# vita-epfl/CrowdNav

Measured on NVIDIA H100. Metric: env-steps/sec at 5 humans × batched envs; 500-case success/collision parity, higher is better.
Workload: dtype f64 state + f32 ORCA solver

## Files before the change

crowdnav_b200/build.py:

```python
#!/usr/bin/env python
import os
import shutil
import subprocess
import sys

HERE = os.path.dirname(os.path.abspath(__file__))
CSRC = os.path.join(HERE, 'csrc')
TARGET = os.path.join(CSRC, 'libcrowdsim_b200.so')
SOURCES = ['step_kernel.cu', 'reset_kernel.cu', 'pack_kernel.cu', 'times_kernel.cu', 'record_kernel.cu']
HEADERS = ['crowdsim_common.cuh', 'orca_device.cuh', 'step_flat.cuh', 'step_multi.cuh', 'step_mid.cuh', 'orca_spec.cuh', 'rotate.cuh', 'step_args.cuh', 'occupancy.cuh', os.path.join('..', '..', 'include', 'crowdsim_b200.h')]
NVCC_FLAGS = ['-gencode', 'arch=compute_90a,code=sm_90a', '-O3', '-lineinfo', '--fmad=false',
              '-prec-div=true', '-prec-sqrt=true', '-ftz=false', '-std=c++17',
              '-Xcompiler', '-fPIC', '-shared', '-cudart', 'shared', '--threads', '4']


def _nvcc():
    for c in (shutil.which('nvcc'), '/usr/local/cuda/bin/nvcc'):
        if c and os.path.exists(c):
            return c
    raise RuntimeError('nvcc not found')


def _stale():
    if not os.path.exists(TARGET):
        return True
    t = os.path.getmtime(TARGET)
    deps = [os.path.join(CSRC, s) for s in SOURCES + HEADERS] + [__file__]
    return any(os.path.exists(d) and os.path.getmtime(d) > t for d in deps)


def build(force=False, verbose=False, extra=()):
    srcs = [os.path.join(CSRC, s) for s in SOURCES]
    if force or _stale():
        cmd = [_nvcc()] + NVCC_FLAGS + list(extra) + srcs + ['-o', TARGET]
        if verbose:
            print(' '.join(cmd))
        subprocess.check_call(cmd)
    return TARGET


if __name__ == '__main__':
    v = '--verbose' in sys.argv
    build(force='--force' in sys.argv, verbose=v, extra=['-Xptxas', '-v'] if v else [])
    print(TARGET)
```

crowdnav_b200/csrc/step_kernel.cu:

```cuda
#include "crowdsim_common.cuh"

namespace cs {

unsigned long long g_launches = 0;
int g_force_generic = 0;

}
#include "step_args.cuh"
#include "step_flat.cuh"
#include "step_multi.cuh"
#include "step_mid.cuh"
namespace cs {

#ifndef CS_MID_MINBLOCKS
#define CS_MID_MINBLOCKS 5
#endif

template <bool MID>
__global__ void __launch_bounds__(MID ? 128 : 256, MID ? CS_MID_MINBLOCKS : 1) step_kernel(const __grid_constant__ StepArgs A)
{
    extern __shared__ __align__(16) unsigned char smem[];
    __shared__ int s_qcount;
    const int T = blockDim.x, tid = threadIdx.x;
    const int N = A.N, L = A.L;
    const KParams &k = A.k;
    const Stage s = carve_stage(smem, A.EPB, L, k.nb_alloc, T);
    if (MID && tid == 0) s_qcount = 0;

    const int le = tid / L, a = tid - le * L;
    const int e = blockIdx.x * A.EPB + le;
    const bool is_robot = (a == N);
    bool live = (e < A.B);
    if (live && A.st.active) live = (A.st.active[e] != 0);

    double2 pos = make_double2(0, 0), vel = pos, goal = pos, attr = pos;
    double theta = 0, gtime = 0;
    if (live) {
        if (!is_robot) {
            const size_t i = (size_t)e * N + a;
            pos = ld2(A.st.h_pos, i); vel = ld2(A.st.h_vel, i); goal = ld2(A.st.h_goal, i); attr = ld2(A.st.h_attr, i);
        } else {
            pos = ld2(A.st.r_pos, e); vel = ld2(A.st.r_vel, e); goal = ld2(A.st.r_goal, e); attr = ld2(A.st.r_attr, e);
            gtime = A.st.g_time[e];
            if (k.robot_policy == CROWDSIM_ROBOT_EXTERNAL_ROT) theta = A.st.r_theta[e];
        }
    }
    stage_agent(s, k, tid, pos, vel, attr.x);
    __syncthreads();

    orca::V2 nv = orca::mk(0.f, 0.f);
    const bool solve = live && (!is_robot || k.robot_policy == CROWDSIM_ROBOT_ORCA) && !(A.act_only && !is_robot);
    if constexpr (MID) nv = mid_solve<kMidM>(s, k, solve, le, a, N, L, pos, goal, attr.y, tid, T, s.lines, &s_qcount);
    else if (solve) nv = orca_predict(s, k, le, a, N, L, pos, goal, attr.y, tid, T);

    if (A.act_only) {
        if (live && is_robot) st2(A.io.action_out, e, make_double2((double)nv.x, (double)nv.y));
        return;
    }

    double ax = 0, ay = 0;
    double2 rvel = make_double2(0, 0);
    if (live && is_robot) {
        if (k.robot_policy == CROWDSIM_ROBOT_ORCA) { ax = (double)nv.x; ay = (double)nv.y; rvel = make_double2(ax, ay); }
        else {
            const double2 act = ld2(A.io.action, e); ax = act.x; ay = act.y;
            if (k.robot_policy == CROWDSIM_ROBOT_EXTERNAL_ROT) rvel = make_double2(ax * cos(ay + theta), ax * sin(ay + theta));
            else rvel = act;
        }
        s.act[le] = rvel;
    }
    __syncthreads();

    const double dt = k.time_step;
    if (live && !is_robot) {
        const double2 rp = s.pos64[le * L + N], ra = s.act[le];
        const double px = pos.x - rp.x, py = pos.y - rp.y;
        const double vx = vel.x - ra.x, vy = vel.y - ra.y;
        const double ex = px + vx * dt, ey = py + vy * dt;
        s.closest[tid] = point_to_segment_dist0(px, py, ex, ey) - attr.x - s.rad64[le * L + N];
    }
    __syncthreads();

    const bool env_ok = (e < A.B);
    int install = 0;
    if (is_robot && env_ok) {
        bool done = false;
        if (live) {
            double dmin = __longlong_as_double(0x7ff0000000000000LL); bool collision = false;
            for (int i = 0; i < N; ++i) {
                const double c = s.closest[le * L + i];
                if (c < 0) { collision = true; break; }
                else if (c < dmin) dmin = c;
            }
            double npx, npy, nvx, nvy;
            if (k.robot_policy != CROWDSIM_ROBOT_EXTERNAL_ROT) { npx = pos.x + ax * dt; npy = pos.y + ay * dt; nvx = ax; nvy = ay; }
            else { const double th = theta + ay; npx = pos.x + cos(th) * ax * dt; npy = pos.y + sin(th) * ax * dt; nvx = nvy = 0; }
            const bool reaching_goal = norm2(npx - goal.x, npy - goal.y) < attr.x;

            double reward; int info;
            if (gtime >= k.time_limit - 1) { reward = 0; done = true; info = CROWDSIM_INFO_TIMEOUT; }
            else if (collision) { reward = k.collision_penalty; done = true; info = CROWDSIM_INFO_COLLISION; }
            else if (reaching_goal) { reward = k.success_reward; done = true; info = CROWDSIM_INFO_REACHGOAL; }
            else if (dmin < k.discomfort_dist) { reward = (dmin - k.discomfort_dist) * k.discomfort_penalty_factor * dt; done = false; info = CROWDSIM_INFO_DANGER; }
            else { reward = 0; done = false; info = CROWDSIM_INFO_NOTHING; }

            if (k.robot_policy == CROWDSIM_ROBOT_EXTERNAL_ROT) {
                double nth = fmod(theta + ay, 2 * CS_PI); if (nth < 0) nth += 2 * CS_PI;
                if (!A.lookahead) A.st.r_theta[e] = nth;
                nvx = ax * cos(nth); nvy = ax * sin(nth);
            }
            const double ntime = gtime + dt;
            if (!A.lookahead) {
                st2(A.st.r_pos, e, make_double2(npx, npy));
                st2(A.st.r_vel, e, make_double2(nvx, nvy));
                A.st.g_time[e] = ntime;
            }
            if (A.io.action_out) st2(A.io.action_out, e, make_double2(nvx, nvy));
            A.io.reward[e] = reward; A.io.dmin[e] = dmin; A.io.done[e] = done ? 1 : 0; A.io.info[e] = (uint8_t)info;

            if (A.has_ep) {
                const crowdsim_episodes &ep = A.ep;
                const int t = ep.ep_steps[e];
                const double disc = (t < ep.discount_len) ? ep.discount[t] : 0.0;
                const double ret = ep.ep_return[e] + disc * reward;
                int tc = ep.ep_too_close[e]; double mds = ep.ep_min_dist_sum[e];
                if (info == CROWDSIM_INFO_DANGER) { tc += 1; mds += dmin; ep.ep_too_close[e] = tc; ep.ep_min_dist_sum[e] = mds; }
                ep.ep_return[e] = ret; ep.ep_steps[e] = t + 1;
                if (done) {
                    const int c = ep.ep_case[e];
                    if (c >= 0) {
                        ep.res_info[c] = (uint8_t)info; ep.res_steps[c] = t + 1;
                        ep.res_time[c] = (info == CROWDSIM_INFO_TIMEOUT) ? k.time_limit : ntime;
                        ep.res_return[c] = ret; ep.res_too_close[c] = tc; ep.res_min_dist_sum[c] = mds;
                        if (ep.res_final_rpos) st2(ep.res_final_rpos, c, make_double2(npx, npy));
                    }
                    if (A.st.active && !A.has_ar) A.st.active[e] = 0;
                }
            }
        }
        if (A.has_ar) install = ar_decide(A, e, ld_relaxed_u8(A.ar.n_state + e), live && done, !live && A.ar.want[e] != 0);
    }
    if (A.has_ar) {
        if (is_robot) s.closest[le * L + N] = (double)install;
        __syncthreads();
        install = (s.closest[le * L + N] != 0.0) && env_ok;
        if (install) {
            if (is_robot) ar_install_robot(A, e);
            else {
                ar_install_human(A, e, N, a);
                if (A.io.obs32) { const double2 np_ = ld2_cg(A.ar.n_h_pos, (size_t)e * N + a); reinterpret_cast<float4 *>(A.io.obs32)[(size_t)e * N + a] = make_float4((float)np_.x, (float)np_.y, 0.f, 0.f); }
            }
        }
        __syncthreads();
        if (install && is_robot) st_release_u8(A.ar.n_state + e, CROWDSIM_SLOT_EMPTY);
    }
    if (live && !is_robot && !install) {
        const double hx = (double)nv.x, hy = (double)nv.y;
        const size_t i = (size_t)e * N + a;
        const double2 np_ = make_double2(pos.x + hx * dt, pos.y + hy * dt);
        if (A.lookahead) { st2(A.la_pos, i, np_); st2(A.la_vel, i, make_double2(hx, hy)); return; }
        st2(A.st.h_pos, i, np_);
        st2(A.st.h_vel, i, make_double2(hx, hy));
        if (A.io.obs32) reinterpret_cast<float4 *>(A.io.obs32)[i] = make_float4((float)np_.x, (float)np_.y, nv.x, nv.y);
    }
}


template <int N>
__global__ void __launch_bounds__(128) orca_act_kernel(const __grid_constant__ StepArgs A)
{
    using namespace orca;
    constexpr int M = N, T = 128;
    __shared__ float s_l[4 * M][T], s_pj[4 * M][T];
    const int e = blockIdx.x * T + threadIdx.x, tid = threadIdx.x;
    if (e >= A.B) return;
    if (A.st.active && !A.st.active[e]) return;
    const KParams &k = A.k;
    const double2 pos = ld2(A.st.r_pos, e), vel = ld2(A.st.r_vel, e), goal = ld2(A.st.r_goal, e), attr = ld2(A.st.r_attr, e);
    const double gvx = goal.x - pos.x, gvy = goal.y - pos.y;
    const double speed = norm2(gvx, gvy);
    const V2 pref = mk((float)((speed > 1) ? gvx / speed : gvx), (float)((speed > 1) ? gvy / speed : gvy));
    const V2 p = mk((float)pos.x, (float)pos.y), v = mk((float)vel.x, (float)vel.y);
    const float r = (float)(attr.x + 0.01 + k.robot_safety_space), max_speed = (float)attr.y;
    V2 hp[M], hv[M]; float hr[M]; float dsq[M]; bool inr[M]; int id[M], src[M];
    #pragma unroll
    for (int c = 0; c < M; ++c) {
        const size_t i = (size_t)e * N + c;
        const double2 q = ld2(A.st.h_pos, i), w = ld2(A.st.h_vel, i), at = ld2(A.st.h_attr, i);
        hp[c] = mk((float)q.x, (float)q.y); hv[c] = mk((float)w.x, (float)w.y); hr[c] = (float)(at.x + 0.01 + k.robot_safety_space);
        dsq[c] = abssq(p - hp[c]); inr[c] = (k.max_neighbors > 0) && dsq[c] < sqr(k.neighbor_dist); id[c] = c;
    }
    int nl = neighbour_order<M>(dsq, inr, id, src);
    nl = nl < k.max_neighbors ? nl : k.max_neighbors;
    RegLines<M> R; bool valid[M];
    #pragma unroll
    for (int kk = 0; kk < M; ++kk) {
        valid[kk] = kk < nl; R.p[kk] = mk(0.f, 0.f); R.d[kk] = mk(0.f, 0.f);
        V2 qp = hp[0], qv = hv[0]; float qr = hr[0];
        #pragma unroll
        for (int c = 1; c < M; ++c) if (src[kk] == c) { qp = hp[c]; qv = hv[c]; qr = hr[c]; }
        if (valid[kk]) make_line_sel(p, v, r, qp, qv, qr, k.inv_time_horizon, k.inv_time_step, R.p[kk], R.d[kk]);
    }
    V2 cand[M]; bool feas[M];
    lp1_all<M, M>(R, valid, max_speed, pref, false, cand, feas);
    V2 nv = mk(0.f, 0.f);
    const int fail = lp2_scan<M, M>(R, valid, nl, cand, feas, lp2_init(pref, max_speed), nv);
    if (fail < nl) {
        const Lines Lr = { &s_l[0][tid], T }, Pr = { &s_pj[0][tid], T };
        #pragma unroll
        for (int kk = 0; kk < M; ++kk) Lr.set(kk, R.p[kk], R.d[kk]);
        lp3(Lr, nl, fail, max_speed, Pr, nv);
    }
    st2(A.io.action_out, e, make_double2((double)nv.x, (double)nv.y));
}

static int sm_count()
{
    static int cache[64];
    int dev = 0; cudaGetDevice(&dev);
    if (dev < 0 || dev >= 64) return 132;
    if (cache[dev] == 0) { int n = 0; cache[dev] = (cudaDeviceGetAttribute(&n, cudaDevAttrMultiProcessorCount, dev) == cudaSuccess && n > 0) ? n : 132; }
    return cache[dev];
}

static int launch(const crowdsim_params *prm, int B, int N, const crowdsim_state *st, const crowdsim_step_io *io,
                  const crowdsim_episodes *ep, const crowdsim_autoreset *ar, int act_only, int n_steps, cudaStream_t stream,
                  double *la_pos = nullptr, double *la_vel = nullptr, const crowdsim_record *rec = nullptr,
                  bool rec_any_route = false, const crowdsim_record_maps *recm = nullptr)
{
    if (!prm || !st || !io || B < 0 || N < 0 || n_steps < 1) return CROWDSIM_EINVAL;
    if (rec) {
        if (rec_any_route ? (N < 1 || N > CROWDSIM_MAX_HUMANS) : (N < 2 || N > 5 || g_force_generic)) return CROWDSIM_EUNSUPPORTED;
        if (prm->robot_policy != CROWDSIM_ROBOT_ORCA) return CROWDSIM_EUNSUPPORTED;
        if (!ep || !ar || !rec->rows || !rec->reward || !rec->t || !rec->code || n_steps > rec->n_max) return CROWDSIM_EINVAL;
        const int rc = check_record_maps(N, recm);
        if (rc != CROWDSIM_OK) return rc;
    }
    if (N > CROWDSIM_MAX_HUMANS || prm->max_neighbors > CROWDSIM_MAX_NEIGHBORS) return CROWDSIM_EUNSUPPORTED;
    if (N > 0 && (!st->h_pos || !st->h_vel || !st->h_goal || !st->h_attr)) return CROWDSIM_EINVAL;
    if (!st->r_pos || !st->r_vel || !st->r_goal || !st->r_attr || !st->g_time) return CROWDSIM_EINVAL;
    if (prm->robot_policy == CROWDSIM_ROBOT_EXTERNAL_ROT && !st->r_theta) return CROWDSIM_EINVAL;
    if (act_only) { if (!io->action_out) return CROWDSIM_EINVAL; }
    else {
        if (!io->reward || !io->dmin || !io->done || !io->info) return CROWDSIM_EINVAL;
        if (prm->robot_policy != CROWDSIM_ROBOT_ORCA && !io->action) return CROWDSIM_EINVAL;
    }
    if (ep && !act_only && (!ep->ep_case || !ep->ep_steps || !ep->ep_return || !ep->ep_too_close || !ep->ep_min_dist_sum ||
                            !ep->discount || !ep->res_info || !ep->res_steps || !ep->res_time || !ep->res_return ||
                            !ep->res_too_close || !ep->res_min_dist_sum)) return CROWDSIM_EINVAL;
    if (ar && !act_only) {
        if (!st->active || !ar->n_state || !ar->n_case || !ar->want || (N > 0 && (!ar->n_h_pos || !ar->n_h_goal || !ar->n_h_attr))) return CROWDSIM_EINVAL;
    }
    if (B == 0) return CROWDSIM_OK;
    StepArgs A;
    A.k = make_kparams(prm, N);
    if (act_only) A.k.robot_policy = CROWDSIM_ROBOT_ORCA;
    A.B = B; A.N = N; A.L = N + 1; A.EPB = envs_per_block(A.L, 128);
    A.st = *st; A.io = *io; A.has_ep = (ep != nullptr && !act_only); A.act_only = act_only; A.n_steps = 1;
    A.lookahead = (la_pos != nullptr); A.la_pos = la_pos; A.la_vel = la_vel;
    if (A.has_ep) A.ep = *ep; else memset(&A.ep, 0, sizeof(A.ep));
    A.has_ar = (ar != nullptr && !act_only);
    if (A.has_ar) A.ar = *ar; else memset(&A.ar, 0, sizeof(A.ar));
    if (rec) A.rec = *rec; else memset(&A.rec, 0, sizeof(A.rec));
    if (recm) A.recm = *recm; else memset(&A.recm, 0, sizeof(A.recm));
    if (act_only && N >= 1 && N <= 5 && !g_force_generic) {
        const int blocks = (B + 127) / 128;
        switch (N) {
            case 1: orca_act_kernel<1><<<blocks, 128, 0, stream>>>(A); break;
            case 2: orca_act_kernel<2><<<blocks, 128, 0, stream>>>(A); break;
            case 3: orca_act_kernel<3><<<blocks, 128, 0, stream>>>(A); break;
            case 4: orca_act_kernel<4><<<blocks, 128, 0, stream>>>(A); break;
            default: orca_act_kernel<5><<<blocks, 128, 0, stream>>>(A); break;
        }
        ++g_launches;
        return (int)cudaGetLastError();
    }
    if ((n_steps > 1 || rec) && N >= 2 && N <= 5 && A.k.robot_policy == CROWDSIM_ROBOT_ORCA && !g_force_generic && !A.lookahead) {
        const int blocks = (B + 31) / 32;
        A.n_steps = n_steps;
        if (rec) { ++g_launches; return launch_multi_record(A, blocks, stream); }
        #define CS_MULTI_LAUNCH(NN) do { if (A.k.robot_visible) step_multi_kernel<NN, true, false><<<blocks, 32 * (NN + 1), 0, stream>>>(A); \
                                         else step_multi_kernel<NN, false, false><<<blocks, 32 * (NN + 1), 0, stream>>>(A); } while (0)
        switch (N) {
            case 2: CS_MULTI_LAUNCH(2); break;
            case 3: CS_MULTI_LAUNCH(3); break;
            case 4: CS_MULTI_LAUNCH(4); break;
            default: CS_MULTI_LAUNCH(5); break;
        }
        #undef CS_MULTI_LAUNCH
        ++g_launches;
        return (int)cudaGetLastError();
    }
    if (N >= 1 && N <= 5 && !g_force_generic && !A.lookahead) {
        const int epb = CS_FLAT_WPB * (32 / (N + 1));
        const int blocks = (B + epb - 1) / epb;
        const bool rot = A.k.robot_policy == CROWDSIM_ROBOT_EXTERNAL_ROT;
        const bool warpq = blocks * CS_FLAT_WPB <= 12 * sm_count();
        #define CS_FLAT_LAUNCH(NN) do { if (rot) step_flat_kernel<NN, 99, true, true><<<blocks, 32 * CS_FLAT_WPB, 0, stream>>>(A); \
                                        else if (warpq) step_flat_kernel<NN, 99, false, true><<<blocks, 32 * CS_FLAT_WPB, 0, stream>>>(A); \
                                        else step_flat_kernel<NN, 99, false, false><<<blocks, 32 * CS_FLAT_WPB, 0, stream>>>(A); } while (0)
        for (int rep = 0; rep < n_steps; ++rep) {
            if (rec) launch_record_between(A, rep - 1, rep, stream);
            switch (N) {
                case 1: CS_FLAT_LAUNCH(1); break;
                case 2: CS_FLAT_LAUNCH(2); break;
                case 3: CS_FLAT_LAUNCH(3); break;
                case 4: CS_FLAT_LAUNCH(4); break;
                default: CS_FLAT_LAUNCH(5); break;
            }
            ++g_launches;
        }
        #undef CS_FLAT_LAUNCH
        if (rec) launch_record_between(A, n_steps - 1, -1, stream);
        return (int)cudaGetLastError();
    }
    const int threads = A.EPB * A.L;
    const int blocks = (B + A.EPB - 1) / A.EPB;
    const bool mid = !g_force_generic && N > 5;
    const size_t smem = mid ? stage_bytes_mid(A.EPB, A.L, mid_lp3_floats()) : stage_bytes(A.EPB, A.L, A.k.nb_alloc, threads);
    if (smem > 48 * 1024) {
        cudaError_t err = mid ? cudaFuncSetAttribute(step_kernel<true>, cudaFuncAttributeMaxDynamicSharedMemorySize, (int)smem)
                              : cudaFuncSetAttribute(step_kernel<false>, cudaFuncAttributeMaxDynamicSharedMemorySize, (int)smem);
        if (err != cudaSuccess) return (int)err;
    }
    for (int rep = 0; rep < n_steps; ++rep) {
        if (rec) launch_record_between(A, rep - 1, rep, stream);
        if (mid) step_kernel<true><<<blocks, threads, smem, stream>>>(A);
        else step_kernel<false><<<blocks, threads, smem, stream>>>(A);
        ++g_launches;
    }
    if (rec) launch_record_between(A, n_steps - 1, -1, stream);
    return (int)cudaGetLastError();
}

}

extern "C" int crowdsim_step(const crowdsim_params *prm, int B, int N, crowdsim_state *st, crowdsim_step_io *io,
                             crowdsim_episodes *ep, const crowdsim_autoreset *ar, void *stream)
{
    return cs::launch(prm, B, N, st, io, ep, ar, 0, 1, (cudaStream_t)stream);
}

extern "C" int crowdsim_step_n(const crowdsim_params *prm, int B, int N, crowdsim_state *st, crowdsim_step_io *io,
                               crowdsim_episodes *ep, const crowdsim_autoreset *ar, int n_steps, void *stream)
{
    return cs::launch(prm, B, N, st, io, ep, ar, 0, n_steps, (cudaStream_t)stream);
}

extern "C" int crowdsim_step_n_record(const crowdsim_params *prm, int B, int N, crowdsim_state *st, crowdsim_step_io *io,
                                      crowdsim_episodes *ep, const crowdsim_autoreset *ar, int n_steps, const crowdsim_record *rec,
                                      void *stream)
{
    if (!rec) return CROWDSIM_EINVAL;
    return cs::launch(prm, B, N, st, io, ep, ar, 0, n_steps, (cudaStream_t)stream, nullptr, nullptr, rec);
}

extern "C" int crowdsim_step_n_record_ex(const crowdsim_params *prm, int B, int N, crowdsim_state *st, crowdsim_step_io *io,
                                         crowdsim_episodes *ep, const crowdsim_autoreset *ar, int n_steps, const crowdsim_record *rec,
                                         const crowdsim_record_maps *maps, void *stream)
{
    if (!rec) return CROWDSIM_EINVAL;
    return cs::launch(prm, B, N, st, io, ep, ar, 0, n_steps, (cudaStream_t)stream, nullptr, nullptr, rec, true, maps);
}

extern "C" int crowdsim_onestep_lookahead(const crowdsim_params *prm, int B, int N, const crowdsim_state *st, crowdsim_step_io *io,
                                          double *next_h_pos, double *next_h_vel, void *stream)
{
    if (!next_h_pos || !next_h_vel || !st) return CROWDSIM_EINVAL;
    if (io && io->obs32) return CROWDSIM_EINVAL;
    return cs::launch(prm, B, N, st, io, nullptr, nullptr, 0, 1, (cudaStream_t)stream, next_h_pos, next_h_vel);
}

extern "C" int crowdsim_orca_act(const crowdsim_params *prm, int B, int N, const crowdsim_state *st, double *action_out,
                                 void *stream)
{
    crowdsim_step_io io; memset(&io, 0, sizeof(io)); io.action_out = action_out;
    return cs::launch(prm, B, N, st, &io, nullptr, nullptr, 1, 1, (cudaStream_t)stream);
}

extern "C" int crowdsim_graph_launch(void *graph_exec, void *stream, void *done_event)
{
    if (!graph_exec) return CROWDSIM_EINVAL;
    cudaError_t e = cudaGraphLaunch((cudaGraphExec_t)graph_exec, (cudaStream_t)stream);
    if (e == cudaSuccess && done_event) e = cudaEventRecord((cudaEvent_t)done_event, (cudaStream_t)stream);
    return (int)e;
}

extern "C" int crowdsim_host_pump(int n, void *const *graph_execs, void *const *graph_execs_alt, int alt_period, int first_round,
                                  void *const *streams, void *const *events,
                                  void *const *copy_dst, const void *const *copy_src, size_t copy_bytes, int rounds)
{
    if (n < 0 || rounds < 0 || !graph_execs || !streams || !events) return CROWDSIM_EINVAL;
    for (int r = 0; r < rounds; ++r)
        for (int i = 0; i < n; ++i) {
            cudaError_t e = cudaEventSynchronize((cudaEvent_t)events[i]);
            if (e != cudaSuccess) return (int)e;
            if (copy_bytes && copy_dst && copy_src && copy_dst[i] && copy_src[i]) memcpy(copy_dst[i], copy_src[i], copy_bytes);
            const bool alt = graph_execs_alt && alt_period > 1 && ((first_round + r) % alt_period) != 0;
            e = cudaGraphLaunch((cudaGraphExec_t)(alt ? graph_execs_alt[i] : graph_execs[i]), (cudaStream_t)streams[i]);
            if (e == cudaSuccess) e = cudaEventRecord((cudaEvent_t)events[i], (cudaStream_t)streams[i]);
            if (e != cudaSuccess) return (int)e;
        }
    return CROWDSIM_OK;
}

extern "C" int crowdsim_event_wait(void *event)
{
    if (!event) return CROWDSIM_EINVAL;
    return (int)cudaEventSynchronize((cudaEvent_t)event);
}

extern "C" void crowdsim_debug_force_generic(int on) { cs::g_force_generic = on; }

extern "C" int crowdsim_abi_version(void) { return CROWDSIM_ABI_VERSION; }

extern "C" unsigned long long crowdsim_launch_count(void) { return cs::g_launches; }

extern "C" int crowdsim_device_check(int *sm_count, int *cc_major, int *cc_minor)
{
    int dev = 0; cudaDeviceProp p;
    if (cudaGetDevice(&dev) != cudaSuccess || cudaGetDeviceProperties(&p, dev) != cudaSuccess) return CROWDSIM_ENODEVICE;
    if (sm_count) *sm_count = p.multiProcessorCount;
    if (cc_major) *cc_major = p.major;
    if (cc_minor) *cc_minor = p.minor;
    return (p.major == 9 && p.minor == 0) ? CROWDSIM_OK : CROWDSIM_ENODEVICE;
}
```

crowdnav_b200/csrc/step_multi.cuh:

```cuda
#pragma once
#include "step_flat.cuh"
#include "rotate.cuh"

namespace cs {

#ifndef CS_MULTI_WARPS
#define CS_MULTI_WARPS 30
#endif

template <int N, int M, bool ROBOT>
__device__ __forceinline__ orca::V2 multi_solve(const KParams &k, const float4 *s_view, const float *s_rview, int ebase, int a,
                                                bool solves, double2 pos, double2 goal, double v_pref, orca::V2 p, orca::V2 v,
                                                float r, const float *s_rl, orca::RegLines<N> &Rq, int &nl_out, int &fail_out,
                                                float &max_speed_out)
{
    using namespace orca;
    const double gvx = goal.x - pos.x, gvy = goal.y - pos.y;
    const double speed = norm2(gvx, gvy);
    const V2 pref = mk((float)((speed > 1) ? gvx / speed : gvx), (float)((speed > 1) ? gvy / speed : gvy));
    const float max_speed = (float)v_pref;

    float dsq[M]; bool inr[M]; int jj[M], src[M];
    #pragma unroll
    for (int c = 0; c < M; ++c) {
        const int j = ROBOT ? c : ((c < N - 1) ? ((c < a) ? c : c + 1) : N);
        jj[c] = j;
        const float4 q = s_view[ebase + j];
        dsq[c] = abssq(p - mk(q.x, q.y));
        inr[c] = solves && (k.max_neighbors > 0) && dsq[c] < sqr(k.neighbor_dist);
    }
    int nl = neighbour_order<M>(dsq, inr, jj, src);
    nl = nl < k.max_neighbors ? nl : k.max_neighbors;

    constexpr int T = 32 * (N + 1);
    if (ROBOT) asm volatile("barrier.sync 1, %0;" :: "r"(T) : "memory");
    RegLines<M> R; bool valid[M];
    #pragma unroll
    for (int kk = 0; kk < M; ++kk) {
        valid[kk] = kk < nl;
        R.p[kk] = mk(0.f, 0.f); R.d[kk] = mk(0.f, 0.f);
        if (valid[kk]) {
            if (ROBOT) {
                const int c = (ebase / (N + 1)) * N + src[kk];
                R.p[kk] = mk(s_rl[0 * T + c], s_rl[1 * T + c]); R.d[kk] = mk(s_rl[2 * T + c], s_rl[3 * T + c]);
            } else {
                const int sl = ebase + src[kk];
                const float4 q = s_view[sl];
                make_line_sel(p, v, r, mk(q.x, q.y), mk(q.z, q.w), s_rview[sl], k.inv_time_horizon, k.inv_time_step, R.p[kk], R.d[kk]);
            }
        }
    }

    V2 cand[M]; bool feas[M];
    lp1_all<M, M>(R, valid, max_speed, pref, false, cand, feas);
    V2 nv = mk(0.f, 0.f);
    fail_out = lp2_scan<M, M>(R, valid, nl, cand, feas, lp2_init(pref, max_speed), nv);
    #pragma unroll
    for (int kk = 0; kk < N; ++kk) { Rq.p[kk] = (kk < M) ? R.p[kk] : mk(0.f, 0.f); Rq.d[kk] = (kk < M) ? R.d[kk] : mk(0.f, 0.f); }
    nl_out = nl; max_speed_out = max_speed;
    return nv;
}

template <int E>
__device__ __forceinline__ float *rec_vpref_smem()
{
    __shared__ float s_vp[E];
    return s_vp;
}

__device__ __forceinline__ void rec_row(const crowdsim_record &rec, int B, int N, int s, int e, int a, double2 hp, double2 hv,
                                        double hr, double2 rp, double2 rv, double2 rg, double rr, float rvp)
{
    float c, sn, rot, dg, rvx, rvy;
    rotate_self((float)rp.x, (float)rp.y, (float)rv.x, (float)rv.y, (float)rg.x, (float)rg.y, c, sn, rot, dg, rvx, rvy);
    float row[13];
    rotate_row(row, (float)rp.x, (float)rp.y, (float)rr, rvp, 0.f, dg, rvx, rvy, c, sn, (float)hp.x, (float)hp.y, (float)hv.x,
               (float)hv.y, (float)hr);
    float *o = rec.rows + (((size_t)s * B + e) * N + a) * 13;
    #pragma unroll
    for (int i = 0; i < 13; ++i) o[i] = row[i];
}

__device__ __forceinline__ void rec_map_state(const crowdsim_record_maps &m, int B, int N, int s, int e, int a, double2 hp, double2 hv)
{
    const size_t i = ((size_t)s * B + e) * N + a;
    st2(m.h_pos, i, hp); st2(m.h_vel, i, hv);
}

template <int N, bool VIS, bool REC>
__global__ void __launch_bounds__(32 * (N + 1), CS_MULTI_WARPS / (N + 1))
step_multi_kernel(const __grid_constant__ StepArgs A)
{
    static_assert(N >= 2 && N <= 5, "small crowds with at least two humans (N = 1 runs n single-step launches)");
    using namespace orca;
    constexpr int E = 32, L = N + 1, T = 32 * L;
    constexpr int MH = VIS ? N : N - 1;
    constexpr int SUB = N - 1;
    constexpr int QC = T / SUB;
    constexpr int QF = 4 * N + 4;
    constexpr int PV = (4 * SUB > 10) ? 4 * SUB : 10;
    __shared__ float s_q[QF][QC];
    __shared__ __align__(16) float s_pv[PV][T];
    __shared__ __align__(16) float s_r2[3][T];
    __shared__ double2 s_pos[T], s_vel[T];
    __shared__ double2 s_goal[T];
    __shared__ double s_rad[T];
    __shared__ float2 s_nv[T];
    __shared__ RobotRec s_rr[E];
    __shared__ uint8_t s_flag[E];
    __shared__ int s_qcount;
    float4 *const s_view = reinterpret_cast<float4 *>(&s_pv[0][0]);
    float *const s_radh = s_pv[4], *const s_radr = s_pv[5];

    const KParams &k = A.k;
    const int tid = threadIdx.x;
    const bool is_robot = tid >= 32 * N;
    const int le = is_robot ? tid - 32 * N : tid / N;
    const int a = is_robot ? N : tid - le * N;
    const int slot_me = le * L + a;
    const int e = blockIdx.x * E + le;
    const bool env_ok = e < A.B;
    const size_t hi = (size_t)e * N + a;
    if (tid == 0) s_qcount = 0;

    double2 pos = make_double2(0, 0), vel = pos, goal = make_double2(3, 4), attr = make_double2(0.3, 1.0);
    uint8_t act_flag = 1;
    if (env_ok) {
        if (A.st.active) act_flag = A.st.active[e];
        if (!is_robot) {
            pos = ld2(A.st.h_pos, hi); vel = ld2(A.st.h_vel, hi); goal = ld2(A.st.h_goal, hi); attr = ld2(A.st.h_attr, hi);
        } else {
            pos = ld2(A.st.r_pos, e); vel = ld2(A.st.r_vel, e); goal = ld2(A.st.r_goal, e); attr = ld2(A.st.r_attr, e);
            RobotRec r0 = {}; r0.ep_c = -1;
            r0.gtime = A.st.g_time[e];
            if (A.has_ep) { r0.ep_t = A.ep.ep_steps[e]; r0.ep_ret = A.ep.ep_return[e]; r0.ep_tc = A.ep.ep_too_close[e]; r0.ep_mds = A.ep.ep_min_dist_sum[e]; r0.ep_c = A.ep.ep_case[e]; }
            if (A.has_ar) r0.want = A.ar.want[e];
            s_rr[le] = r0;
        }
    }
    s_goal[tid] = goal;
    RobotRec &rr = s_rr[le];

    bool dirty_kin = false, dirty_scene = false;
    bool release = false;
    const double dt = k.time_step;

    #pragma unroll 1
    for (int s = 0; ; ++s) {
    const bool live = env_ok && (act_flag != 0);
    const float fpx = (float)pos.x, fpy = (float)pos.y, fvx = (float)vel.x, fvy = (float)vel.y;
    const float frh = (float)(attr.x + 0.01 + k.human_safety_space);
    const float frr = (float)(attr.x + 0.01 + k.robot_safety_space);
    s_view[slot_me] = make_float4(fpx, fpy, fvx, fvy); s_radh[slot_me] = frh; s_radr[slot_me] = frr;
    s_pos[tid] = pos; s_vel[tid] = vel; s_rad[tid] = attr.x;
    if constexpr (REC) { if (is_robot) rec_vpref_smem<E>()[le] = (float)attr.y; }
    const bool work = live || (is_robot && env_ok && A.has_ar && rr.want != 0);
    const int go = __syncthreads_or(s < A.n_steps && work);
    if (release) { st_release_u8(A.ar.n_state + e, CROWDSIM_SLOT_EMPTY); release = false; }
    if (!go) {
        if constexpr (REC) { if (is_robot && env_ok) for (int s2 = s; s2 < A.n_steps; ++s2) A.rec.code[(size_t)s2 * A.B + e] = CROWDSIM_REC_NONE; }
        break;
    }
    if constexpr (REC) {
        if (!is_robot && live) {
            const int rt = 32 * N + le;
            rec_row(A.rec, A.B, N, s, e, a, pos, vel, attr.x, s_pos[rt], s_vel[rt], s_goal[rt], s_rad[rt], rec_vpref_smem<E>()[le]);
            if (A.recm.h_pos) rec_map_state(A.recm, A.B, N, s, e, a, pos, vel);
        }
    }

    const V2 p = mk(fpx, fpy), v = mk(fvx, fvy);
    if (!is_robot) {
        const int rs = le * L + N;
        const float4 q = s_view[rs];
        V2 lp, ld;
        make_line_sel(mk(q.x, q.y), mk(q.z, q.w), s_radr[rs], p, v, frr, k.inv_time_horizon, k.inv_time_step, lp, ld);
        s_pv[6][tid] = lp.x; s_pv[7][tid] = lp.y; s_pv[8][tid] = ld.x; s_pv[9][tid] = ld.y;
        asm volatile("barrier.arrive 1, %0;" :: "r"(T) : "memory");
    }
    RegLines<N> R; int nl, fail; float max_speed;
    V2 nv = is_robot ? multi_solve<N, N, true>(k, s_view, s_radr, le * L, N, live, pos, s_goal[tid], attr.y, p, v, frr, s_pv[6], R, nl, fail, max_speed)
                     : multi_solve<N, MH, false>(k, s_view, s_radh, le * L, a, live, pos, s_goal[tid], attr.y, p, v, frh, s_pv[6], R, nl, fail, max_speed);

    const bool pending = live && fail < nl;
    int slot = pending ? atomicAdd(&s_qcount, 1) : -1;
    if (slot >= QC) {
        float lq[4 * N], lp[4 * SUB];
        #pragma unroll
        for (int kk = 0; kk < N; ++kk) { lq[4 * kk + 0] = R.p[kk].x; lq[4 * kk + 1] = R.p[kk].y; lq[4 * kk + 2] = R.d[kk].x; lq[4 * kk + 3] = R.d[kk].y; }
        const Lines Lq = { lq, 1 }, Pq = { lp, 1 };
        lp3(Lq, nl, fail, max_speed, Pq, nv);
        slot = -1;
    } else if (slot >= 0) {
        #pragma unroll
        for (int kk = 0; kk < N; ++kk) {
            s_q[4 * kk + 0][slot] = R.p[kk].x; s_q[4 * kk + 1][slot] = R.p[kk].y; s_q[4 * kk + 2][slot] = R.d[kk].x; s_q[4 * kk + 3][slot] = R.d[kk].y;
        }
        s_q[4 * N + 0][slot] = __int_as_float(nl); s_q[4 * N + 1][slot] = __int_as_float(fail);
        s_q[4 * N + 2][slot] = max_speed; s_q[4 * N + 3][slot] = __int_as_float(tid);
    }
    s_nv[tid] = make_float2(nv.x, nv.y);
    const int cnt = __syncthreads_count(slot >= 0);
    if (cnt > 0) {
        if (tid == 0) s_qcount = 0;
        const int item = tid / SUB, i = tid % SUB + 1;
        const bool mine = (tid < QC * SUB) && item < cnt;
        if (mine) {
            const Lines Lq = { &s_q[0][item], QC };
            const int qn = __float_as_int(s_q[4 * N + 0][item]);
            bool ok = false; V2 r2 = mk(0.f, 0.f);
            if (i < qn) {
                const Lines Pq = { &s_pv[0][tid], T };
                ok = lp3_subproblem(Lq, i, s_q[4 * N + 2][item], Pq, r2);
            }
            s_r2[0][tid] = r2.x; s_r2[1][tid] = r2.y; s_r2[2][tid] = ok ? 1.0f : 0.0f;
        }
        __syncthreads();
        if (mine && i == 1) {
            const Lines Lq = { &s_q[0][item], QC };
            const int qn = __float_as_int(s_q[4 * N + 0][item]), qf = __float_as_int(s_q[4 * N + 1][item]);
            const float qr = s_q[4 * N + 2][item];
            const int owner = __float_as_int(s_q[4 * N + 3][item]);
            const float2 r0 = s_nv[owner];
            V2 res = mk(r0.x, r0.y);
            lp3_outer_scan(Lq, qn, qf, qr, res, [&](int ii, V2 &r2) {
                const int src_ = tid + (ii - 1);
                r2 = mk(s_r2[0][src_], s_r2[1][src_]);
                return s_r2[2][src_] != 0.0f;
            });
            s_nv[owner] = make_float2(res.x, res.y);
        }
        __syncthreads();
        if (slot >= 0) { const float2 q = s_nv[tid]; nv = mk(q.x, q.y); }
    }
    pos = s_pos[tid]; vel = s_vel[tid];

    double *const s_cl = reinterpret_cast<double *>(&s_r2[0][0]);
    if (!is_robot) {
        if (live) {
            const int rt = 32 * N + le;
            const float2 rv = s_nv[rt];
            const double2 rp = s_pos[rt];
            const double px = pos.x - rp.x, py = pos.y - rp.y;
            const double vx = vel.x - (double)rv.x, vy = vel.y - (double)rv.y;
            const double ex = px + vx * dt, ey = py + vy * dt;
            s_cl[tid] = point_to_segment_dist0(px, py, ex, ey) - attr.x - s_rad[rt];
            const double hx = (double)nv.x, hy = (double)nv.y;
            pos = make_double2(pos.x + hx * dt, pos.y + hy * dt); vel = make_double2(hx, hy);
            dirty_kin = true;
        }
    }
    __syncthreads();
    if (is_robot) {
        int install = 0;
        if (env_ok) {
            bool done = false;
            if (live) {
                const double ax = (double)nv.x, ay = (double)nv.y;
                double dmin = __longlong_as_double(0x7ff0000000000000LL); bool collision = false;
                #pragma unroll
                for (int i = 0; i < N; ++i) {
                    const double ci = s_cl[le * N + i];
                    if (!collision) { if (ci < 0) collision = true; else if (ci < dmin) dmin = ci; }
                }
                const double npx = pos.x + ax * dt, npy = pos.y + ay * dt;
                const double2 goal = s_goal[tid];
                const bool reaching_goal = norm2(npx - goal.x, npy - goal.y) < attr.x;
                double reward; int info;
                const double gtime = rr.gtime;
                const int t_rec = rr.ep_t;
                if (gtime >= k.time_limit - 1) { reward = 0; done = true; info = CROWDSIM_INFO_TIMEOUT; }
                else if (collision) { reward = k.collision_penalty; done = true; info = CROWDSIM_INFO_COLLISION; }
                else if (reaching_goal) { reward = k.success_reward; done = true; info = CROWDSIM_INFO_REACHGOAL; }
                else if (dmin < k.discomfort_dist) { reward = (dmin - k.discomfort_dist) * k.discomfort_penalty_factor * dt; done = false; info = CROWDSIM_INFO_DANGER; }
                else { reward = 0; done = false; info = CROWDSIM_INFO_NOTHING; }
                pos = make_double2(npx, npy); vel = make_double2(ax, ay);
                const double ntime = gtime + dt;
                rr.gtime = ntime;
                rr.o_act = vel; rr.o_reward = reward; rr.o_dmin = dmin; rr.o_done = done ? 1 : 0; rr.o_info = info; rr.any_live = 1;
                dirty_kin = true;
                if (A.has_ep) {
                    const crowdsim_episodes &ep = A.ep;
                    int ep_t = rr.ep_t, ep_tc = rr.ep_tc; double ep_ret = rr.ep_ret, ep_mds = rr.ep_mds;
                    const double disc = (ep_t < ep.discount_len) ? ep.discount[ep_t] : 0.0;
                    ep_ret = ep_ret + disc * reward; ep_t += 1;
                    if (info == CROWDSIM_INFO_DANGER) { ep_tc += 1; ep_mds += dmin; }
                    rr.ep_t = ep_t; rr.ep_tc = ep_tc; rr.ep_ret = ep_ret; rr.ep_mds = ep_mds;
                    rr.dirty_ep = 1;
                    if (done) {
                        const int ep_c = rr.ep_c;
                        if (ep_c >= 0) {
                            ep.res_info[ep_c] = (uint8_t)info; ep.res_steps[ep_c] = ep_t;
                            ep.res_time[ep_c] = (info == CROWDSIM_INFO_TIMEOUT) ? k.time_limit : ntime;
                            ep.res_return[ep_c] = ep_ret; ep.res_too_close[ep_c] = ep_tc; ep.res_min_dist_sum[ep_c] = ep_mds;
                            if (ep.res_final_rpos) st2(ep.res_final_rpos, ep_c, pos);
                        }
                        if (A.st.active && !A.has_ar) { A.st.active[e] = 0; act_flag = 0; }
                    }
                }
                if constexpr (REC) {
                    const size_t ri = (size_t)s * A.B + e;
                    A.rec.reward[ri] = reward; A.rec.t[ri] = t_rec;
                    A.rec.code[ri] = !done ? CROWDSIM_REC_LIVE : (info == CROWDSIM_INFO_TIMEOUT) ? CROWDSIM_REC_DROPPED : CROWDSIM_REC_STORED;
                }
            } else if constexpr (REC) {
                A.rec.code[(size_t)s * A.B + e] = CROWDSIM_REC_NONE;
            }
            if (A.has_ar) {
                const bool finished = live && done, parked = !live && rr.want != 0;
                if (finished || parked) {
                    const uint8_t sst = ld_relaxed_u8(A.ar.n_state + e);
                    if (sst == CROWDSIM_SLOT_READY) install = 1;
                    else {
                        act_flag = 0; A.st.active[e] = 0;
                        const uint8_t want = (sst == CROWDSIM_SLOT_EXHAUSTED) ? 0 : 1;
                        rr.want = want; A.ar.want[e] = want;
                    }
                }
                if (install) {
                    (void)ld_acquire_u8(A.ar.n_state + e);
                    pos = make_double2(0.0, -A.ar.circle_radius); s_goal[tid] = make_double2(0.0, A.ar.circle_radius);
                    vel = make_double2(0, 0); attr = make_double2(A.ar.robot_radius, A.ar.robot_v_pref);
                    rr.gtime = 0.0;
                    if (A.st.r_theta) A.st.r_theta[e] = CS_PI / 2;
                    if (A.has_ep) { rr.ep_t = 0; rr.ep_ret = 0.0; rr.ep_tc = 0; rr.ep_mds = 0.0; rr.ep_c = __ldcg(A.ar.n_case + e); rr.dirty_ep = 1; rr.new_case = 1; }
                    act_flag = 1; A.st.active[e] = 1; rr.want = 0; A.ar.want[e] = 0;
                    dirty_kin = true; dirty_scene = true; release = true;
                }
            }
        }
        s_flag[le] = (uint8_t)((act_flag != 0) | (install << 1));
    }
    __syncthreads();
    if (!is_robot) {
        const unsigned f = s_flag[le];
        act_flag = (uint8_t)(f & 1u);
        if ((f & 2u) && env_ok) {
            (void)ld_acquire_u8(A.ar.n_state + e);
            pos = ld2_cg(A.ar.n_h_pos, hi); vel = make_double2(0, 0); s_goal[tid] = ld2_cg(A.ar.n_h_goal, hi); attr = ld2_cg(A.ar.n_h_attr, hi);
            dirty_kin = true; dirty_scene = true;
        }
    }
    }

    if (env_ok) {
        if (!is_robot) {
            if (dirty_kin) {
                st2(A.st.h_pos, hi, pos); st2(A.st.h_vel, hi, vel);
                if (A.io.obs32) reinterpret_cast<float4 *>(A.io.obs32)[hi] = make_float4((float)pos.x, (float)pos.y, (float)vel.x, (float)vel.y);
            }
            if (dirty_scene) { st2(A.st.h_goal, hi, s_goal[tid]); st2(A.st.h_attr, hi, attr); }
        } else {
            if (dirty_kin) { st2(A.st.r_pos, e, pos); st2(A.st.r_vel, e, vel); A.st.g_time[e] = rr.gtime; }
            if (dirty_scene) { st2(A.st.r_goal, e, s_goal[tid]); st2(A.st.r_attr, e, attr); }
            if (rr.any_live) {
                if (A.io.action_out) st2(A.io.action_out, e, rr.o_act);
                A.io.reward[e] = rr.o_reward; A.io.dmin[e] = rr.o_dmin; A.io.done[e] = rr.o_done; A.io.info[e] = (uint8_t)rr.o_info;
            }
            if (A.has_ep && rr.dirty_ep) {
                A.ep.ep_steps[e] = rr.ep_t; A.ep.ep_return[e] = rr.ep_ret; A.ep.ep_too_close[e] = rr.ep_tc; A.ep.ep_min_dist_sum[e] = rr.ep_mds;
                if (rr.new_case) A.ep.ep_case[e] = rr.ep_c;
            }
        }
    }
}

}
```

Baseline: 1.189 billion.

## Remove per-step block barriers by precomputing done flags and warp-local queue solves

Restructures the multi-env step loop so the robot publishes timeout, goal, slot-ready and want flags before the existing barrier. Human threads then derive done and auto-reset decisions themselves, which removes the second block-wide __syncthreads per step. The deferred-solve queue is remapped so each item's sub-threads sit in one warp, letting a __syncwarp replace a block barrier. Global loads (slot state, discount) are hoisted earlier to overlap the barrier, and an optional clock64 phase probe is added behind a compile flag, with the risk that the humans' duplicated done logic drifts from the robot's.

```diff
diff --git a/crowdnav_b200/build.py b/crowdnav_b200/build.py
--- a/crowdnav_b200/build.py
+++ b/crowdnav_b200/build.py
@@ -21,25 +21,33 @@
     raise RuntimeError('nvcc not found')
 
 
-def _stale():
-    if not os.path.exists(TARGET):
+def _stale(target):
+    if not os.path.exists(target):
         return True
-    t = os.path.getmtime(TARGET)
+    t = os.path.getmtime(target)
     deps = [os.path.join(CSRC, s) for s in SOURCES + HEADERS] + [__file__]
     return any(os.path.exists(d) and os.path.getmtime(d) > t for d in deps)
 
 
-def build(force=False, verbose=False, extra=()):
+def build(force=False, verbose=False, extra=(), out=None):
+    target = os.path.abspath(out) if out else TARGET
     srcs = [os.path.join(CSRC, s) for s in SOURCES]
-    if force or _stale():
-        cmd = [_nvcc()] + NVCC_FLAGS + list(extra) + srcs + ['-o', TARGET]
+    if force or _stale(target):
+        os.makedirs(os.path.dirname(target), exist_ok=True)
+        cmd = [_nvcc()] + NVCC_FLAGS + list(extra) + srcs + ['-o', target]
         if verbose:
             print(' '.join(cmd))
         subprocess.check_call(cmd)
-    return TARGET
+    return target
 
 
 if __name__ == '__main__':
-    v = '--verbose' in sys.argv
-    build(force='--force' in sys.argv, verbose=v, extra=['-Xptxas', '-v'] if v else [])
-    print(TARGET)
+    import argparse
+    ap = argparse.ArgumentParser()
+    ap.add_argument('--force', action='store_true')
+    ap.add_argument('--verbose', action='store_true')
+    ap.add_argument('--out', default=None, help='output path (default: %s)' % TARGET)
+    ap.add_argument('-D', dest='defines', action='append', default=[], help='preprocessor define, e.g. CS_PHASE_PROBE')
+    a = ap.parse_args()
+    extra = ['-D' + d for d in a.defines] + (['-Xptxas', '-v'] if a.verbose else [])
+    print(build(force=a.force or bool(a.defines), verbose=a.verbose, extra=extra, out=a.out))
diff --git a/crowdnav_b200/csrc/step_kernel.cu b/crowdnav_b200/csrc/step_kernel.cu
--- a/crowdnav_b200/csrc/step_kernel.cu
+++ b/crowdnav_b200/csrc/step_kernel.cu
@@ -416,6 +416,19 @@
 
 extern "C" unsigned long long crowdsim_launch_count(void) { return cs::g_launches; }
 
+#ifdef CS_PHASE_PROBE
+extern "C" int crowdsim_phase_probe(unsigned long long *out, int reset)
+{
+    cudaError_t e = cudaDeviceSynchronize();
+    if (e == cudaSuccess && out) e = cudaMemcpyFromSymbol(out, cs::g_phase, sizeof(cs::g_phase));
+    if (e == cudaSuccess && reset) {
+        static const unsigned long long zero[2][CS_PHASES + 1] = {};
+        e = cudaMemcpyToSymbol(cs::g_phase, zero, sizeof(zero));
+    }
+    return (int)e;
+}
+#endif
+
 extern "C" int crowdsim_device_check(int *sm_count, int *cc_major, int *cc_minor)
 {
     int dev = 0; cudaDeviceProp p;
diff --git a/crowdnav_b200/csrc/step_multi.cuh b/crowdnav_b200/csrc/step_multi.cuh
--- a/crowdnav_b200/csrc/step_multi.cuh
+++ b/crowdnav_b200/csrc/step_multi.cuh
@@ -6,6 +6,20 @@
 
 #ifndef CS_MULTI_WARPS
 #define CS_MULTI_WARPS 30
+#endif
+
+#define CS_PHASES 8
+#ifdef CS_PHASE_PROBE
+static __device__ unsigned long long g_phase[2][CS_PHASES + 1];
+#define CS_PROBE_INIT unsigned ph_acc[CS_PHASES] = {}; long long ph_t = clock64();
+#define CS_PROBE(i) do { const long long t_ = clock64(); ph_acc[i] += (unsigned)(t_ - ph_t); ph_t = t_; } while (0)
+#define CS_PROBE_FLUSH(robot, steps) do { if ((threadIdx.x & 31) == 0) {                                                    \
+        for (int i_ = 0; i_ < CS_PHASES; ++i_) atomicAdd(&g_phase[(robot) ? 1 : 0][i_], (unsigned long long)ph_acc[i_]);    \
+        atomicAdd(&g_phase[(robot) ? 1 : 0][CS_PHASES], (unsigned long long)(steps)); } } while (0)
+#else
+#define CS_PROBE_INIT
+#define CS_PROBE(i) do { } while (0)
+#define CS_PROBE_FLUSH(robot, steps) do { } while (0)
 #endif
 
 template <int N, int M, bool ROBOT>
@@ -96,7 +110,8 @@
     constexpr int E = 32, L = N + 1, T = 32 * L;
     constexpr int MH = VIS ? N : N - 1;
     constexpr int SUB = N - 1;
-    constexpr int QC = T / SUB;
+    constexpr int IPW = 32 / SUB;
+    constexpr int QC = IPW * L;
     constexpr int QF = 4 * N + 4;
     constexpr int PV = (4 * SUB > 10) ? 4 * SUB : 10;
     __shared__ float s_q[QF][QC];
@@ -107,8 +122,9 @@
     __shared__ double s_rad[T];
     __shared__ float2 s_nv[T];
     __shared__ RobotRec s_rr[E];
-    __shared__ uint8_t s_flag[E];
+    __shared__ uint8_t s_pre[E];
     __shared__ int s_qcount;
+    constexpr unsigned PRE_TIMEOUT = 1, PRE_GOAL = 2, PRE_READY = 4, PRE_WANT = 8;
     float4 *const s_view = reinterpret_cast<float4 *>(&s_pv[0][0]);
     float *const s_radh = s_pv[4], *const s_radr = s_pv[5];
 
@@ -144,6 +160,7 @@
     bool dirty_kin = false, dirty_scene = false;
     bool release = false;
     const double dt = k.time_step;
+    CS_PROBE_INIT
 
     #pragma unroll 1
     for (int s = 0; ; ++s) {
@@ -159,8 +176,10 @@
     if (release) { st_release_u8(A.ar.n_state + e, CROWDSIM_SLOT_EMPTY); release = false; }
     if (!go) {
         if constexpr (REC) { if (is_robot && env_ok) for (int s2 = s; s2 < A.n_steps; ++s2) A.rec.code[(size_t)s2 * A.B + e] = CROWDSIM_REC_NONE; }
+        CS_PROBE_FLUSH(is_robot, s);
         break;
     }
+    CS_PROBE(0);
     if constexpr (REC) {
         if (!is_robot && live) {
             const int rt = 32 * N + le;
@@ -200,11 +219,19 @@
         s_q[4 * N + 2][slot] = max_speed; s_q[4 * N + 3][slot] = __int_as_float(tid);
     }
     s_nv[tid] = make_float2(nv.x, nv.y);
+    uint8_t sst = CROWDSIM_SLOT_EMPTY;
+    double disc = 0.0;
+    if (is_robot && env_ok) {
+        if (A.has_ar) sst = ld_relaxed_u8(A.ar.n_state + e);
+        if (A.has_ep && live) { const int t = rr.ep_t; disc = (t < A.ep.discount_len) ? A.ep.discount[t] : 0.0; }
+    }
+    CS_PROBE(1);
     const int cnt = __syncthreads_count(slot >= 0);
+    CS_PROBE(2);
     if (cnt > 0) {
         if (tid == 0) s_qcount = 0;
-        const int item = tid / SUB, i = tid % SUB + 1;
-        const bool mine = (tid < QC * SUB) && item < cnt;
+        const int lane = tid & 31, item = (tid >> 5) * IPW + lane / SUB, i = lane % SUB + 1;
+        const bool mine = lane < IPW * SUB && item < cnt;
         if (mine) {
             const Lines Lq = { &s_q[0][item], QC };
             const int qn = __float_as_int(s_q[4 * N + 0][item]);
@@ -215,7 +242,7 @@
             }
             s_r2[0][tid] = r2.x; s_r2[1][tid] = r2.y; s_r2[2][tid] = ok ? 1.0f : 0.0f;
         }
-        __syncthreads();
+        __syncwarp();
         if (mine && i == 1) {
             const Lines Lq = { &s_q[0][item], QC };
             const int qn = __float_as_int(s_q[4 * N + 0][item]), qf = __float_as_int(s_q[4 * N + 1][item]);
@@ -234,8 +261,10 @@
         if (slot >= 0) { const float2 q = s_nv[tid]; nv = mk(q.x, q.y); }
     }
     pos = s_pos[tid]; vel = s_vel[tid];
+    CS_PROBE(3);
 
     double *const s_cl = reinterpret_cast<double *>(&s_r2[0][0]);
+    bool timeout = false, reaching_goal = false;
     if (!is_robot) {
         if (live) {
             const int rt = 32 * N + le;
@@ -249,10 +278,41 @@
             pos = make_double2(pos.x + hx * dt, pos.y + hy * dt); vel = make_double2(hx, hy);
             dirty_kin = true;
         }
-    }
+    } else if (env_ok) {
+        if (live) {
+            const double npx = pos.x + (double)nv.x * dt, npy = pos.y + (double)nv.y * dt;
+            const double2 goal = s_goal[tid];
+            reaching_goal = norm2(npx - goal.x, npy - goal.y) < attr.x;
+            timeout = rr.gtime >= k.time_limit - 1;
+        }
+        s_pre[le] = (uint8_t)((timeout ? PRE_TIMEOUT : 0u) | (reaching_goal ? PRE_GOAL : 0u) |
+                              (sst == CROWDSIM_SLOT_READY ? PRE_READY : 0u) | (rr.want != 0 ? PRE_WANT : 0u));
+    }
+    CS_PROBE(4);
     __syncthreads();
-    if (is_robot) {
-        int install = 0;
+    CS_PROBE(5);
+    if (!is_robot) {
+        if (env_ok) {
+            const unsigned pf = s_pre[le];
+            bool done = false;
+            if (live) {
+                bool collision = false;
+                #pragma unroll
+                for (int i = 0; i < N; ++i) collision |= s_cl[le * N + i] < 0;
+                done = (pf & PRE_TIMEOUT) || collision || (pf & PRE_GOAL);
+                if (done && A.has_ep && A.st.active && !A.has_ar) act_flag = 0;
+            }
+            if (A.has_ar && ((live && done) || (!live && (pf & PRE_WANT)))) {
+                act_flag = (pf & PRE_READY) ? 1 : 0;
+                if (act_flag) {
+                    (void)ld_acquire_u8(A.ar.n_state + e);
+                    pos = ld2_cg(A.ar.n_h_pos, hi); vel = make_double2(0, 0); s_goal[tid] = ld2_cg(A.ar.n_h_goal, hi); attr = ld2_cg(A.ar.n_h_attr, hi);
+                    dirty_kin = true; dirty_scene = true;
+                }
+            }
+        }
+        CS_PROBE(6);
+    } else {
         if (env_ok) {
             bool done = false;
             if (live) {
@@ -264,12 +324,10 @@
                     if (!collision) { if (ci < 0) collision = true; else if (ci < dmin) dmin = ci; }
                 }
                 const double npx = pos.x + ax * dt, npy = pos.y + ay * dt;
-                const double2 goal = s_goal[tid];
-                const bool reaching_goal = norm2(npx - goal.x, npy - goal.y) < attr.x;
                 double reward; int info;
                 const double gtime = rr.gtime;
                 const int t_rec = rr.ep_t;
-                if (gtime >= k.time_limit - 1) { reward = 0; done = true; info = CROWDSIM_INFO_TIMEOUT; }
+                if (timeout) { reward = 0; done = true; info = CROWDSIM_INFO_TIMEOUT; }
                 else if (collision) { reward = k.collision_penalty; done = true; info = CROWDSIM_INFO_COLLISION; }
                 else if (reaching_goal) { reward = k.success_reward; done = true; info = CROWDSIM_INFO_REACHGOAL; }
                 else if (dmin < k.discomfort_dist) { reward = (dmin - k.discomfort_dist) * k.discomfort_penalty_factor * dt; done = false; info = CROWDSIM_INFO_DANGER; }
@@ -282,7 +340,6 @@
                 if (A.has_ep) {
                     const crowdsim_episodes &ep = A.ep;
                     int ep_t = rr.ep_t, ep_tc = rr.ep_tc; double ep_ret = rr.ep_ret, ep_mds = rr.ep_mds;
-                    const double disc = (ep_t < ep.discount_len) ? ep.discount[ep_t] : 0.0;
                     ep_ret = ep_ret + disc * reward; ep_t += 1;
                     if (info == CROWDSIM_INFO_DANGER) { ep_tc += 1; ep_mds += dmin; }
                     rr.ep_t = ep_t; rr.ep_tc = ep_tc; rr.ep_ret = ep_ret; rr.ep_mds = ep_mds;
@@ -309,37 +366,24 @@
             if (A.has_ar) {
                 const bool finished = live && done, parked = !live && rr.want != 0;
                 if (finished || parked) {
-                    const uint8_t sst = ld_relaxed_u8(A.ar.n_state + e);
-                    if (sst == CROWDSIM_SLOT_READY) install = 1;
-                    else {
+                    if (sst == CROWDSIM_SLOT_READY) {
+                        (void)ld_acquire_u8(A.ar.n_state + e);
+                        pos = make_double2(0.0, -A.ar.circle_radius); s_goal[tid] = make_double2(0.0, A.ar.circle_radius);
+                        vel = make_double2(0, 0); attr = make_double2(A.ar.robot_radius, A.ar.robot_v_pref);
+                        rr.gtime = 0.0;
+                        if (A.st.r_theta) A.st.r_theta[e] = CS_PI / 2;
+                        if (A.has_ep) { rr.ep_t = 0; rr.ep_ret = 0.0; rr.ep_tc = 0; rr.ep_mds = 0.0; rr.ep_c = __ldcg(A.ar.n_case + e); rr.dirty_ep = 1; rr.new_case = 1; }
+                        act_flag = 1; A.st.active[e] = 1; rr.want = 0; A.ar.want[e] = 0;
+                        dirty_kin = true; dirty_scene = true; release = true;
+                    } else {
                         act_flag = 0; A.st.active[e] = 0;
                         const uint8_t want = (sst == CROWDSIM_SLOT_EXHAUSTED) ? 0 : 1;
                         rr.want = want; A.ar.want[e] = want;
                     }
                 }
-                if (install) {
-                    (void)ld_acquire_u8(A.ar.n_state + e);
-                    pos = make_double2(0.0, -A.ar.circle_radius); s_goal[tid] = make_double2(0.0, A.ar.circle_radius);
-                    vel = make_double2(0, 0); attr = make_double2(A.ar.robot_radius, A.ar.robot_v_pref);
-                    rr.gtime = 0.0;
-                    if (A.st.r_theta) A.st.r_theta[e] = CS_PI / 2;
-                    if (A.has_ep) { rr.ep_t = 0; rr.ep_ret = 0.0; rr.ep_tc = 0; rr.ep_mds = 0.0; rr.ep_c = __ldcg(A.ar.n_case + e); rr.dirty_ep = 1; rr.new_case = 1; }
-                    act_flag = 1; A.st.active[e] = 1; rr.want = 0; A.ar.want[e] = 0;
-                    dirty_kin = true; dirty_scene = true; release = true;
-                }
-            }
-        }
-        s_flag[le] = (uint8_t)((act_flag != 0) | (install << 1));
-    }
-    __syncthreads();
-    if (!is_robot) {
-        const unsigned f = s_flag[le];
-        act_flag = (uint8_t)(f & 1u);
-        if ((f & 2u) && env_ok) {
-            (void)ld_acquire_u8(A.ar.n_state + e);
-            pos = ld2_cg(A.ar.n_h_pos, hi); vel = make_double2(0, 0); s_goal[tid] = ld2_cg(A.ar.n_h_goal, hi); attr = ld2_cg(A.ar.n_h_attr, hi);
-            dirty_kin = true; dirty_scene = true;
-        }
+            }
+        }
+        CS_PROBE(6);
     }
     }
 
```

Measured after the change: 1.230 billion (median of 6 runs). +3.5%, better.
